# dontLoveBugs/CSPN_monodepth

Hardware: AMD Instinct MI355X
Metric: depth-maps/sec at 304x228 b=24, 24 CSPN iters (higher is better)
Workload: dtype f32

## Files before the change

### cspn_monodepth_amd/_lib.py

```python
import ctypes
import os
import shutil
import subprocess
import threading

_PKG = os.path.dirname(os.path.abspath(__file__))
_ROOT = os.path.dirname(_PKG)
SO_PATH = os.environ.get("CSPN_HIP_LIB") or os.path.join(_PKG, "libcspn_hip.so")
CSRC = os.path.join(_PKG, "csrc")
SOURCES = ("cspn_propagate.hip", "cspn_resident.hip", "cspnk_resident.hip", "cspnk_d2.hip", "cspn_prepare.hip", "cspn_backward.hip", "cspn_metrics.hip", "cspn_metrics_frame.hip", "cspn_debug.hip", "cspn_repair.hip", "pac_conv2d.hip", "pac_conv2d_s2.hip", "cspn_unpool.hip")
HEADERS = (os.path.join(CSRC, "cspn_common.hpp"), os.path.join(CSRC, "cspnk_helpers.hpp"), os.path.join(_ROOT, "include", "cspn_hip.h"))
INCLUDE = os.path.join(_ROOT, "include")

CSPN_F32, CSPN_F16 = 0, 1
ABI_VERSION = 10
BLEND_NONE, BLEND_SPARSE, BLEND_PREMASK = 0, 1, 2

EXPORTS = (
    "cspn_abi_version", "cspn_last_error", "cspn_plan_resolve", "cspn3_prepare", "cspn_pac_prepare",
    "cspn_propagate_workspace_bytes", "cspn_propagate", "cspn_propagate_scored", "cspn_propagate_transposed", "cspn3_propagate_from_guidance",
    "cspn_transpose_weights", "cspn3_resident_plan", "cspn3_resident_workspace_bytes", "cspn3_forward_resident", "cspn3_transposed_resident", "cspn3_transposed_resident_guidance",
    "cspnk_resident_plan", "cspnk_resident_workspace_bytes", "cspnk_forward_resident", "cspnk_forward_resident_history", "cspnk_transposed_resident",
    "cspn_grad_weights", "cspn3_grad_guidance", "cspn_pac_grad_guided", "cspn3_backward_tail",
    "cspn_pac_backward_tail", "cspn_metrics_accumulate", "cspn_metrics_per_frame_workspace_bytes", "cspn_metrics_per_frame", "cspn_meter_update",
    "cspn_pac_out_size", "cspn_pac_force_generic", "cspn_pac_conv2d", "cspn_pac_conv2d_grad_input", "cspn_pac_conv2d_grad_kernel", "cspn_pac_nd2col", "cspn_unpool2d", "cspn_unpool2d_backward", "cspn_debug_set_lds_poison",
)


class cspn_plan(ctypes.Structure):
    _fields_ = [("steps_per_launch", ctypes.c_int), ("tile_w", ctypes.c_int), ("tile_h", ctypes.c_int),
                ("quads_per_thread", ctypes.c_int), ("threads", ctypes.c_int), ("force_scalar", ctypes.c_int)]


class cspn_resident_plan(ctypes.Structure):
    _fields_ = [(n, ctypes.c_int) for n in ("steps_per_phase", "tiles_x", "tiles_y", "tile_w", "tile_h", "quads_per_thread",
                                            "threads", "images_per_launch", "launches", "lds_bytes", "n_cu")] + \
               [("region_over_tile", ctypes.c_float), ("spin_limit", ctypes.c_uint), ("debug_stamps", ctypes.c_void_p),
                ("step_form", ctypes.c_int), ("guard", ctypes.c_int)]


STEP_AUTO, STEP_FMA, STEP_DOT2 = 0, 1, 2


class cspn_conv_geometry(ctypes.Structure):
    _fields_ = [(n, ctypes.c_int) for n in ("kh", "kw", "sh", "sw", "ph", "pw", "dh", "dw", "oph", "opw", "transposed")]


BENCH_UNRELATED = ("pac_conv2d.hip", "pac_conv2d_s2.hip", "cspn_unpool.hip", "cspn_metrics_frame.hip")


def _source_digest(flags, code_only=False):
    import hashlib
    import re
    h = hashlib.sha256(" ".join(flags).encode())
# ... 51 lines not shown
        objs = list(pool.map(compile_one, srcs))
    cmd = [hipcc, "--offload-arch=gfx950", "-shared", "-fPIC", "-o", SO_PATH + ".tmp"] + objs
    if verbose:
        print(" ".join(cmd), flush=True)
    subprocess.check_call(cmd)
    os.replace(SO_PATH + ".tmp", SO_PATH)
    with open(stamp, "w") as fh:
        fh.write(digest + "\n")
    return SO_PATH


_lib = None
_lock = threading.Lock()


def _declare(lib):
    vp, ci, cl, cs = ctypes.c_void_p, ctypes.c_int, ctypes.c_long, ctypes.c_size_t
    lib.cspn_abi_version.restype = ci
    lib.cspn_last_error.restype = ctypes.c_char_p
    lib.cspn_plan_resolve.argtypes = [ci, ci, ci, ci, ci, ci, ctypes.POINTER(cspn_plan), ctypes.POINTER(cspn_plan)]
    lib.cspn3_prepare.argtypes = [vp, ci, cl, cl, ci, ci, ci, ci, vp, ci, vp, vp]
    lib.cspn_pac_prepare.argtypes = [vp, ci, ci, ci, ci, ci, vp, ci, vp]
    lib.cspn_propagate_workspace_bytes.argtypes = [ci, ci, ci, ci, ci, ci]
    lib.cspn_propagate_workspace_bytes.restype = cs
    lib.cspn_propagate.argtypes = [vp, ci, vp, vp, vp, vp, vp, ci, ci, ci, ci, ci, ci, ci, ci,
                                   ctypes.POINTER(cspn_plan), vp]
    lib.cspn_propagate_scored.argtypes = [vp, ci, vp, vp, vp, vp, ci, ci, ci, ci, ci, ci, ci, ci, vp, vp, ci,
                                          ctypes.POINTER(cspn_plan), vp]
    lib.cspn_propagate_transposed.argtypes = [vp, ci, vp, vp, vp, ci, ci, ci, ci, ci, ci, ci, ctypes.POINTER(cspn_plan), vp]
    lib.cspn3_propagate_from_guidance.argtypes = [vp, ci, cl, cl, vp, vp, vp, vp, vp, vp, vp, ci, ci, ci, ci, ci, ci, ci,
                                                  vp, vp, ci,
                                                  ctypes.POINTER(cspn_plan), vp]
    lib.cspn3_resident_plan.argtypes = [ci, ci, ci, ci, ci, ci, ctypes.POINTER(cspn_resident_plan)]
    lib.cspn3_resident_workspace_bytes.argtypes = [ci, ci, ci]
    lib.cspn3_resident_workspace_bytes.restype = cs
    lib.cspn3_forward_resident.argtypes = [vp, cl, cl, vp, vp, vp, vp, vp, vp, vp, ctypes.c_uint, vp, ci, ci, ci, ci, ci, ci, vp, vp, ci,
                                           ctypes.POINTER(cspn_resident_plan), vp]
    lib.cspn3_transposed_resident.argtypes = [vp, vp, vp, vp, vp, ctypes.c_uint, vp, ci, ci, ci, ci, ci, ci,
                                              ctypes.POINTER(cspn_resident_plan), vp]
    lib.cspn3_transposed_resident_guidance.argtypes = [vp, cl, cl, vp, vp, vp, vp, vp, ctypes.c_uint, vp, ci, ci, ci, ci, ci, ci,
                                                       ctypes.POINTER(cspn_resident_plan), vp]
    lib.cspnk_resident_plan.argtypes = [ci, ci, ci, ci, ci, ci, ci, ci, ctypes.POINTER(cspn_resident_plan)]
    lib.cspnk_resident_workspace_bytes.argtypes = [ci, ci, ci, ci]
    lib.cspnk_resident_workspace_bytes.restype = cs
    lib.cspnk_forward_resident.argtypes = [vp, ci, ci, vp, vp, vp, ci, vp, ctypes.c_uint, vp, ci, ci, ci, ci, ci, vp, vp, ci,
                                           ctypes.POINTER(cspn_resident_plan), vp]
    lib.cspnk_forward_resident_history.argtypes = [vp, ci, ci, vp, vp, vp, vp, vp, ctypes.c_uint, vp, ci, ci, ci, ci, ci,
                                                   ctypes.POINTER(cspn_resident_plan), vp]
    lib.cspnk_transposed_resident.argtypes = [vp, ci, ci, vp, vp, ci, vp, vp, vp, ctypes.c_uint, vp, ci, ci, ci, ci, ci,
                                              ctypes.POINTER(cspn_resident_plan), vp]
    lib.cspn_transpose_weights.argtypes = [vp, vp, ci, ci, ci, ci, ci, vp]
    lib.cspn_grad_weights.argtypes = [vp, vp, vp, vp, vp, vp, vp, ci, ci, ci, ci, ci, ci, vp]
    lib.cspn3_grad_guidance.argtypes = [vp, ci, cl, cl, ci, vp, ci, vp, vp, vp, ci, ci, ci, vp]
    lib.cspn_pac_grad_guided.argtypes = [vp, ci, vp, vp, ci, ci, ci, ci, ci, vp]
    lib.cspn3_backward_tail.argtypes = [vp, vp, vp, vp, vp, vp, cl, cl, ci, vp, vp, vp, vp, ci, ci, ci, ci, ci, vp]
    lib.cspn_pac_backward_tail.argtypes = [vp, vp, vp, vp, vp, vp, vp, vp, ci, ci, ci, ci, ci, ci, ci, ci, vp]
    lib.cspn_metrics_accumulate.argtypes = [vp, vp, ci, cs, vp, ci, vp]
    lib.cspn_metrics_per_frame_workspace_bytes.argtypes = [ci, cs]
    lib.cspn_metrics_per_frame_workspace_bytes.restype = cs
    lib.cspn_metrics_per_frame.argtypes = [vp, vp, ci, ci, cs, vp, vp, vp]
    lib.cspn_meter_update.argtypes = [vp, ci, vp, vp]
    geom = ctypes.POINTER(cspn_conv_geometry)
    lib.cspn_pac_out_size.argtypes = [ci, ci, geom, ctypes.POINTER(ci), ctypes.POINTER(ci)]
    lib.cspn_pac_force_generic.argtypes = [ci, ctypes.POINTER(ci)]
    lib.cspn_pac_conv2d.argtypes = [vp, vp, vp, ci, ci, ci, ci, ci, ci, geom, vp]
    lib.cspn_pac_conv2d_grad_input.argtypes = [vp, vp, vp, ci, ci, ci, ci, ci, ci, geom, vp]
# ... 35 lines not shown
```

### cspn_monodepth_amd/csrc/cspn_resident.hip

```cpp
#include "cspn_common.hpp"

#include <atomic>

namespace {

struct ResArgs {
    const float* g;
    long g_bs, g_cs;
    const float* d0;
    const float* sparse;
    float* out;
    float* xbuf;
    unsigned* flags;
    unsigned* status;
    unsigned* host_err;
    int last_chunk;
    unsigned seq;
    float* hist;
    float* w_out;
    float* s_out;
    const float* s_in;
    const float* target;
    double* macc;
    int nslots;
    int B, H, W, Wv, T, S;
    int tw, th, tiles_x, tiles_y;
    int wq, wr, hxw, hyw, dr, ls;
    int b0, nb;
    unsigned spin_limit;
    unsigned long long* dbg;
};

__device__ __forceinline__ void st4_dev(float* base, unsigned elem, float a, float b, float c, float d) {
    const v4f v = {a, b, c, d};
    asm volatile("global_store_dwordx4 %0, %1, %2 sc1" ::"v"(elem * 4u), "v"(v), "s"(base) : "memory");
}
template <typename T>
__device__ __forceinline__ T* uniform_ptr(T* p) {
    const unsigned long long u = reinterpret_cast<unsigned long long>(p);
    const unsigned lo = __builtin_amdgcn_readfirstlane((unsigned)u), hi = __builtin_amdgcn_readfirstlane((unsigned)(u >> 32));
    return reinterpret_cast<T*>(((unsigned long long)hi << 32) | lo);
}
#define GLB __attribute__((address_space(1)))
typedef GLB char* gptr;
__device__ __forceinline__ gptr at32(const float* base, unsigned e) {
    return (gptr) reinterpret_cast<unsigned long long>(base) + (e << 2);
}
__device__ __forceinline__ float4 ld4(gptr p) {
    const v4f v = *reinterpret_cast<const GLB v4f*>(p);
    return make_float4(v.x, v.y, v.z, v.w);
}
__device__ __forceinline__ float ld1(gptr p) { return *reinterpret_cast<const GLB float*>(p); }
__device__ __forceinline__ void st4(gptr p, float4 v) {
    const v4f w = {v.x, v.y, v.z, v.w};
    *reinterpret_cast<GLB v4f*>(p) = w;
}
#ifndef CSPN_RES_HIST_NT
#define CSPN_RES_HIST_NT 1
#endif
#ifndef CSPN_RES_STEP_PIPE
#define CSPN_RES_STEP_PIPE 0
#endif
#ifndef CSPN_RES_PUBLISH_ALL
#define CSPN_RES_PUBLISH_ALL 1
#endif
__device__ __forceinline__ void st4_hist(gptr p, float4 v) {
    const v4f w = {v.x, v.y, v.z, v.w};
    if (CSPN_RES_HIST_NT) __builtin_nontemporal_store(w, reinterpret_cast<GLB v4f*>(p));
    else *reinterpret_cast<GLB v4f*>(p) = w;
}
__device__ __forceinline__ float4 ld4_dev(gptr p) {
    const unsigned long long lo = __hip_atomic_load(reinterpret_cast<const GLB unsigned long long*>(p), __ATOMIC_RELAXED, __HIP_MEMORY_SCOPE_AGENT);
    const unsigned long long hi = __hip_atomic_load(reinterpret_cast<const GLB unsigned long long*>(p) + 1, __ATOMIC_RELAXED, __HIP_MEMORY_SCOPE_AGENT);
    return make_float4(__uint_as_float((unsigned)lo), __uint_as_float((unsigned)(lo >> 32)), __uint_as_float((unsigned)hi),
                       __uint_as_float((unsigned)(hi >> 32)));
}
__device__ __forceinline__ float ld1_dev(gptr p) {
    return __uint_as_float(__hip_atomic_load(reinterpret_cast<const GLB unsigned*>(p), __ATOMIC_RELAXED, __HIP_MEMORY_SCOPE_AGENT));
}

constexpr int RES_THREADS = 512;
constexpr int RES_PP = 16352;

template <int NQ, int NTHREADS, int BLEND, int MODE, int CLEAN, int PAC = 0>
__global__ __launch_bounds__(NTHREADS, NTHREADS / 256) void cspn3_resident(const ResArgs a) {
    static_assert(!PAC || MODE <= 2, "the softmax-weight form has no transposed sweep of its own (the published volume feeds MODE 3)");
    constexpr int R = 1, NT = 8, WIN = 6;
    constexpr bool SCORE = MODE == 1, TRANSG = MODE == 4, TRANS = MODE == 3 || TRANSG, HIST = MODE == 2 || TRANS;
    extern __shared__ __attribute__((aligned(16))) float lds[];
    __shared__ int wg_bad;

    const int tid = threadIdx.x;
    const int tiles_per_img = a.tiles_x * a.tiles_y;
    const int wg_round = a.nb * tiles_per_img;
    const int round = (int)blockIdx.x / wg_round;
    const int tile = xcd_contiguous_id((int)blockIdx.x - round * wg_round, wg_round);
    const int bl = tile / tiles_per_img;
// ... 14 lines not shown
            const unsigned old = __hip_atomic_fetch_add(a.status + 2, 1u, __ATOMIC_RELAXED, __HIP_MEMORY_SCOPE_AGENT);
            if (old + 1u == gridDim.x) {
                __hip_atomic_store(a.status + 2, 0u, __ATOMIC_RELAXED, __HIP_MEMORY_SCOPE_AGENT);
                if (a.host_err && a.last_chunk) __hip_atomic_store(a.host_err + 1, a.seq, __ATOMIC_RELAXED, __HIP_MEMORY_SCOPE_SYSTEM);
            }
        }
    };

    if (b >= a.B) { count_out(); return; }

    const float* __restrict__ din0 = uniform_ptr(a.d0 + (size_t)b * HW);
    const float* __restrict__ spg = BLEND ? uniform_ptr(a.sparse + (size_t)b * HW) : nullptr;

    const int wq = a.wq, wr = a.wr;
    const int sy = tid / wq;
    const int sx = tid - sy * wq;
    const int r0 = sy * NQ;
    const bool exch = a.T > a.S;
    const int rx0 = max(exch ? max(0, x0 - a.tw) : 0, min(x0 - a.hxw, W - 4 * wq));
    const int ry0 = max(exch ? max(0, y0 - a.th) : 0, min(y0 - a.hyw, H - wr));
    const int xq = rx0 + 4 * sx;
    const int yq0 = ry0 + r0;
    const bool x_in = (xq >= 0) && (xq < a.Wv);
    const int nval = a.Wv - xq;
    const int lane = tid & 63;
    const bool fix_left = (sx == 0) || (lane == 0);
    const bool fix_right = (sx == wq - 1) || (lane == 63);

    const int dr = a.dr, ls = a.ls;
    float* const cur = lds;
    float* const nxt = lds + RES_PP;
    const int yd0 = ry0 - R;
    const int xd0 = rx0 - 4;
    float4 st0[NQ + 1];
    unsigned st0_in = 0;
    const int step_r = NTHREADS / wq, step_q = NTHREADS - step_r * wq;
    {
    int row = sy, qx = sx;
#pragma unroll
    for (int u = 0; u <= NQ; ++u) {
        const int y = yd0 + row, x = xd0 + 4 + 4 * qx;
        const bool valid = row < dr;
        const bool in = valid && (y >= 0 && y < H && x >= 0 && x < a.Wv);
        if (in) st0_in |= 1u << u;
        st0[u] = ld4(at32(din0, in ? (unsigned)(y * W + x) : 0u));
        if (TRANS && BLEND) {
            const float4 sp = ld4(at32(spg, in ? (unsigned)(y * W + x) : 0u));
            st0[u].x *= 1.f - sgnf(sp.x); st0[u].y *= 1.f - sgnf(sp.y); st0[u].z *= 1.f - sgnf(sp.z); st0[u].w *= 1.f - sgnf(sp.w);
        }
        row += step_r; qx += step_q;
        if (qx >= wq) { qx -= wq; ++row; }
    }
    }
    float ring0 = 0.f;
    bool ring0_in = false;
    if (tid < dr * 2 * R) {
        const int row = tid / (2 * R), c = tid - row * (2 * R);
        const int lc = (c < R) ? (4 - R + c) : (4 + 4 * wq + (c - R));
        const int y = yd0 + row, x = xd0 + lc;
        ring0_in = (y >= 0 && y < H && x >= 0 && x < a.Wv);
        ring0 = ld1(at32(din0, ring0_in ? (unsigned)(y * W + x) : 0u));
        if (TRANS && BLEND) ring0 *= 1.f - sgnf(ld1(at32(spg, ring0_in ? (unsigned)(y * W + x) : 0u)));
    }

    float wreg[NQ][NT][4];
    unsigned in_img = 0, interior = 0;
// ... 204 lines not shown
    float* hist_step = HIST ? uniform_ptr(a.hist + (size_t)b * HW) : nullptr;
    const int n_phase = (a.T + a.S - 1) / a.S;
    const int tile_global = b * tiles_per_img + trem;
    float own[NQ][4];
    float nbl[NQ], nbr[NQ];

    for (int p = 0; p < n_phase; ++p) {
        const int steps = (a.T - p * a.S) < a.S ? (a.T - p * a.S) : a.S;
        const bool last_phase = (p == n_phase - 1);
        const float* __restrict__ xin = uniform_ptr(a.xbuf + (size_t)((p + 1) & 1) * plane + (size_t)b * HW);
        if (p > 0) {
            int tidp = tid;
            asm volatile("" : "+v"(tidp));
            const int tq_in = min(a.tw, rx0 + 4 * wq - x0) >> 2;
            const int th_in = min(a.th, ry0 + wr - y0);
            const int nl = (x0 - rx0) >> 2;
            const int nside = wq - tq_in;
            const int nrow_t = (y0 - ry0) + R;
            const int n_top = nrow_t * wq;
            const int n_bot = (dr - nrow_t - th_in) * wq;
            const int n_side = th_in * nside;
            const int n_halo = n_top + n_bot + n_side;
            float ring_v = 0.f;
            int ring_at = -1;
            if (tidp < dr * 2 * R) {
                const int row = tidp / (2 * R), c = tidp - row * (2 * R);
                const int lc = (c < R) ? (4 - R + c) : (4 + 4 * wq + (c - R));
                const int y = yd0 + row, x = xd0 + lc;
                const bool in = (y >= 0 && y < H && x >= 0 && x < a.Wv);
                const float v = ld1_dev(at32(xin, in ? (unsigned)(y * W + x) : 0u));
                ring_v = in ? v : 0.f;
                ring_at = row * ls + lc;
            }
            for (int base = 0; base < n_halo; base += 2 * NTHREADS) {
                float4 hv[2];
                int at[2];
#pragma unroll
                for (int u = 0; u < 2; ++u) {
                    const int h = base + u * NTHREADS + tidp;
                    int row, qx;
                    if (h < n_top) { row = h / wq; qx = h - row * wq; }
                    else if (h < n_top + n_bot) { const int h2 = h - n_top; row = h2 / wq; qx = h2 - row * wq; row += nrow_t + th_in; }
                    else {
                        const int h3 = h - n_top - n_bot;
                        const int ns = nside > 0 ? nside : 1;
                        row = h3 / ns;
                        const int c = h3 - row * ns;
                        row += nrow_t;
                        qx = c < nl ? c : c + tq_in;
                    }
                    const int y = yd0 + row, x = xd0 + 4 + 4 * qx;
                    const bool valid = h < n_halo;
                    const bool in = valid && y >= 0 && y < H && x >= 0 && x < a.Wv;
                    const float4 v = ld4_dev(at32(xin, in ? (unsigned)(y * W + x) : 0u));
                    hv[u] = make_float4(in ? v.x : 0.f, in ? v.y : 0.f, in ? v.z : 0.f, in ? v.w : 0.f);
                    at[u] = valid ? row * ls + 4 + 4 * qx : -1;
                }
#pragma unroll
                for (int u = 0; u < 2; ++u)
                    if (at[u] >= 0) *reinterpret_cast<float4*>(&cur[at[u]]) = hv[u];
            }
            if (ring_at >= 0) { cur[ring_at] = ring_v; nxt[ring_at] = 0.f; }
            for (int c = tidp; c < 2 * ls; c += NTHREADS) nxt[(c < ls ? 0 : (dr - 1) * ls - ls) + c] = 0.f;
        }
        __syncthreads();

#pragma unroll
        for (int i = 0; i < NQ; ++i) {
            int drow = r0L + i + R;
            drow = drow < dr ? drow : dr - 1;
            const v4f mid = *(lds_cv4f_ptr)(cur + drow * ls + cb);
            own[i][0] = mid.x; own[i][1] = mid.y; own[i][2] = mid.z; own[i][3] = mid.w;
        }
        if (CSPN_RES_STEP_PIPE) {
#pragma unroll
            for (int i = 0; i < NQ; ++i) { nbl[i] = dpp_from_prev_lane(own[i][3]); nbr[i] = dpp_from_next_lane(own[i][0]); }
        }
        if (BLEND && !TRANS && p == 0) {
#pragma unroll
            for (int i = 0; i < NQ; ++i) {
                if (r0L + i < wr) {
                    float4* slot = reinterpret_cast<float4*>(md_lds + (tid * NQ + i) * 4);
                    const float4 m = *slot;
                    *slot = make_float4(m.x * own[i][0], m.y * own[i][1], m.z * own[i][2], m.w * own[i][3]);
                }
            }
        }
        auto step = [&](auto final_c, auto on_c, auto par_c, int final_par) __attribute__((always_inline)) {
            constexpr bool FINAL = decltype(final_c)::value;
            constexpr int PAR = decltype(par_c)::value;
// ... 147 lines not shown
            if (s < plain_steps) step(std::false_type{}, std::true_type{}, P0{}, 0);
            if (last_phase) step(std::true_type{}, std::true_type{}, P0{}, plain_steps & 1);
        } else {
            for (int s = 0; s < plain_steps; ++s) step(std::false_type{}, std::false_type{}, P0{}, 0);
            if (last_phase) step(std::true_type{}, std::false_type{}, P0{}, 0);
        }
        stamp();
        if (!last_phase) {
            float* __restrict__ xout = uniform_ptr(a.xbuf + (size_t)(p & 1) * plane + (size_t)b * HW);
            if (active) {
                unsigned o0 = (unsigned)(yq0L * W + xqL);
                asm volatile("" : "+v"(o0));
#if !CSPN_RES_PUBLISH_ALL
                auto reg_x0 = [&](int t) { const int xx0 = t * a.tw; return max(max(0, xx0 - a.tw), min(xx0 - a.hxw, W - 4 * wq)); };
                auto reg_y0 = [&](int t) { const int yy0 = t * a.th; return max(max(0, yy0 - a.th), min(yy0 - a.hyw, H - wr)); };
                const int pubL = tx > 0 ? reg_x0(tx - 1) + 4 * wq + 1 : -(1 << 30);
                const int pubR = tx + 1 < a.tiles_x ? reg_x0(tx + 1) - 1 : (1 << 30);
                const int pubT = ty > 0 ? reg_y0(ty - 1) + wr + 1 : -(1 << 30);
                const int pubB = ty + 1 < a.tiles_y ? reg_y0(ty + 1) - 1 : (1 << 30);
                const bool col_read = (xqL < pubL) || (xqL + 3 >= pubR);
#endif
#pragma unroll
                for (int i = 0; i < NQ; ++i) {
#if !CSPN_RES_PUBLISH_ALL
                    const bool read = col_read || (yq0L + i < pubT) || (yq0L + i >= pubB);
#else
                    const bool read = true;
#endif
                    if (((interior >> i) & 1u) && read) st4_dev(xout, o0 + (unsigned)(i * W), own[i][0], own[i][1], own[i][2], own[i][3]);
                }
            }
            asm volatile("s_waitcnt vmcnt(0)" ::: "memory");
            __syncthreads();
            const unsigned want = a.seq + (unsigned)p + 1u;
            if (tid == 0) __hip_atomic_store(a.flags + tile_global, want, __ATOMIC_RELAXED, __HIP_MEMORY_SCOPE_AGENT);
            if (tid < 9 && tid != 4) {
                const int ny = ty + tid / 3 - 1, nx = tx + tid % 3 - 1;
                if (ny >= 0 && ny < a.tiles_y && nx >= 0 && nx < a.tiles_x) {
                    const gptr f = (gptr) reinterpret_cast<unsigned long long>(uniform_ptr(a.flags)) + ((unsigned)(b * tiles_per_img + ny * a.tiles_x + nx) << 2);
                    unsigned spins = 0;
                    while ((int)(__hip_atomic_load(reinterpret_cast<const GLB unsigned*>(f), __ATOMIC_RELAXED, __HIP_MEMORY_SCOPE_AGENT) - want) < 0) {
                        ++spins;
                        if ((spins & 255u) == 0u && __hip_atomic_load(a.status, __ATOMIC_RELAXED, __HIP_MEMORY_SCOPE_AGENT) == a.seq) {
                            wg_bad = 1;
                            break;
                        }
                        if (spins >= a.spin_limit) {
                            __hip_atomic_store(a.status, a.seq, __ATOMIC_RELAXED, __HIP_MEMORY_SCOPE_AGENT);
                            wg_bad = 1;
                            break;
                        }
                        __builtin_amdgcn_s_sleep(2);
                    }
                }
            }
            __syncthreads();
            stamp();
            if (wg_bad) {
                if (tid == 0) {
                    __hip_atomic_store(a.status + 1, 1u, __ATOMIC_RELAXED, __HIP_MEMORY_SCOPE_AGENT);
                    if (a.host_err) __hip_atomic_store(a.host_err, 1u, __ATOMIC_RELAXED, __HIP_MEMORY_SCOPE_SYSTEM);
                    __atomic_thread_fence(__ATOMIC_SEQ_CST);
                }
                {
                    const float qnan = __uint_as_float(CSPN_POISON_F32);
                    float* const pz = HIST ? uniform_ptr(a.hist + (size_t)(a.T - 1) * plane + (size_t)b * HW) : dout;
                    unsigned o0 = (unsigned)(yq0L * W + xqL);
                    asm volatile("" : "+v"(o0));
#pragma unroll
                    for (int i = 0; i < NQ; ++i)
                        if ((interior >> i) & 1u) st4(at32(pz, o0 + (unsigned)(i * W)), make_float4(qnan, qnan, qnan, qnan));
                }
                count_out();
                return;
            }
        }
    }
    if (SCORE) {
        float mf[10];
#pragma unroll
        for (int k = 0; k < 10; ++k) mf[k] = 0.f;
        if (active) {
            float4 scored_t[NQ];
            const float* tgt_b = uniform_ptr(a.target + (size_t)b * HW);
            unsigned o0s = (unsigned)(yq0L * W + xqL);
// ... 30 lines not shown
        }
    }
    count_out();
}

constexpr int RES_MAX_NQ = 5;

constexpr int RES_MAX_ROUNDS = 8;
#ifndef CSPN_RES_ONE_LAUNCH
#define CSPN_RES_ONE_LAUNCH 0
#endif
struct ResGeom {
    int S, tiles_x, tiles_y, tw, th, nq, wq, wr, hxw, hyw, dr, ls;
    int imgs_per_launch, launches;
    size_t lds_bytes;
    double cost;
    int threads = RES_THREADS;
};

int cu_count() {
    static std::atomic<int> cached[64];
    int dev = 0;
    if (hipGetDevice(&dev) != hipSuccess) return 0;
    int n = cached[dev & 63].load(std::memory_order_relaxed);
    if (n > 0) return n;
    hipDeviceProp_t prop;
    if (hipGetDeviceProperties(&prop, dev) != hipSuccess) return 0;
    cached[dev & 63].store(prop.multiProcessorCount, std::memory_order_relaxed);
    return prop.multiProcessorCount;
}

size_t res_lds_bytes(int dr, int ls, int nq, int blend, int threads = RES_THREADS) {
    return ((size_t)RES_PP + (size_t)dr * ls + (size_t)(blend ? 1 : 0) * threads * nq * 4 + 16 * 10) * sizeof(float);
}

#ifndef CSPN_RES_LS_SWIZZLE
#define CSPN_RES_LS_SWIZZLE 1
#endif
int res_row_stride(int wq, int nq, int dr) {
    const int lo = 4 * wq + 8;
    if (!CSPN_RES_LS_SWIZZLE) return lo;
    for (int cand = lo; cand < lo + 64; cand += 4)
        if ((((nq * cand - 4 * wq) % 64) + 64) % 64 == 0 && (size_t)dr * cand <= (size_t)RES_PP) return cand;
    return lo;
}

bool regions_inside_image(const ResGeom& g, int H, int W, int Wv, int T) {
    if (Wv != W) return false;
    const bool exch = T > g.S;
    for (int tx = 0; tx < g.tiles_x; ++tx) {
        const int x0 = tx * g.tw;
        int rx0 = x0 - g.hxw; if (rx0 > W - 4 * g.wq) rx0 = W - 4 * g.wq;
        int lo = exch ? x0 - g.tw : 0; if (lo < 0) lo = 0;
        if (rx0 < lo) rx0 = lo;
        if (rx0 + 4 * g.wq > W) return false;
    }
    for (int ty = 0; ty < g.tiles_y; ++ty) {
        const int y0 = ty * g.th;
        int ry0 = y0 - g.hyw; if (ry0 > H - g.wr) ry0 = H - g.wr;
        int lo = exch ? y0 - g.th : 0; if (lo < 0) lo = 0;
        if (ry0 < lo) ry0 = lo;
        if (ry0 + g.wr > H) return false;
    }
    return true;
}

// ... 79 lines not shown
        if (mode == 2) return launch_resident_inst<NQ, 1, 2, CLEAN>(a, grid, lds, st);
        return mode ? launch_resident_inst<NQ, 1, 1, CLEAN>(a, grid, lds, st) : launch_resident_inst<NQ, 1, 0, CLEAN>(a, grid, lds, st);
    }
    if (mode == 2) return launch_resident_inst<NQ, 0, 2, CLEAN>(a, grid, lds, st);
    return mode ? launch_resident_inst<NQ, 0, 1, CLEAN>(a, grid, lds, st) : launch_resident_inst<NQ, 0, 0, CLEAN>(a, grid, lds, st);
}
template <int NQ>
int launch_resident_nq(const ResArgs& a, int grid, size_t lds, int blend, int mode, bool clean, hipStream_t st) {
    return clean ? launch_resident_c<NQ, 1>(a, grid, lds, blend, mode, st) : launch_resident_c<NQ, 0>(a, grid, lds, blend, mode, st);
}


}

namespace {
int resident_launch(const void* guidance, long bs, long cs, const void* d0, const void* sparse, void* out, void* history,
                    void* w8_out, float* s_out, void* work, unsigned seq, unsigned* host_err, int B, int H, int W, int W_valid,
                    int T, int blend, const void* target, double* acc, int nslots, const cspn_resident_plan* plan,
                    cspn_stream_t stream, bool transposed, bool pac = false, const float* s_in = nullptr);
}

extern "C" {

int cspn3_resident_plan(int B, int H, int W, int T, int blend, int n_cu, cspn_resident_plan* out) {
    if (!out || B < 1 || H < 1 || W < 1 || T < 0) return fail("cspn3_resident_plan: bad arguments");
    if (n_cu <= 0) n_cu = cu_count();
    if (n_cu <= 0) return fail("cspn3_resident_plan: no device (pass n_cu > 0 to plan without one)");
    ResGeom g;
    if (T < 1 || !resident_geometry(B, H, W, T, blend, n_cu, out->steps_per_phase, &g, out->threads))
        return fail("cspn3_resident_plan: no resident tiling for B=%d %dx%d T=%d on %d CUs (W %% 4 == 0 needed)", B, H, W, T, n_cu);
    if (ceil_div(T, g.S) > 255) return fail("cspn3_resident_plan: T=%d in %d-step phases is more than 255 phases", T, g.S);
    out->steps_per_phase = g.S; out->tiles_x = g.tiles_x; out->tiles_y = g.tiles_y; out->tile_w = g.tw; out->tile_h = g.th;
    out->quads_per_thread = g.nq; out->threads = g.threads; out->images_per_launch = g.imgs_per_launch;
    out->launches = g.launches; out->lds_bytes = (int)g.lds_bytes; out->n_cu = n_cu;
    out->region_over_tile = (float)((double)(4 * g.wq) * g.wr / ((double)g.tw * g.th));
    return 1;
}

size_t cspn3_resident_workspace_bytes(int B, int H, int W) {
    const size_t planes = (size_t)2 * B * H * W * sizeof(float);
    const size_t flags = ((size_t)B * (((size_t)H * W) / 16 + 1) + 4) * sizeof(unsigned);
    return ((planes + 15) & ~(size_t)15) + ((flags + 15) & ~(size_t)15);
}

int cspn3_forward_resident(const void* guidance, long bs, long cs, const void* d0, const void* sparse, void* out,
                           void* history, void* w8_out, float* s_out,
                           void* work, unsigned seq, unsigned* host_err, int B, int H, int W, int W_valid, int T, int blend,
                           const void* target, double* acc, int nslots, const cspn_resident_plan* plan,
                           cspn_stream_t stream) {
    return resident_launch(guidance, bs, cs, d0, sparse, out, history, w8_out, s_out, work, seq, host_err, B, H, W, W_valid, T,
                           blend, target, acc, nslots, plan, stream, false);
}

int cspn3_transposed_resident(const void* w8, const float* g_T, const float* sparse_f32, float* history, void* work,
                              unsigned seq, unsigned* host_err, int B, int H, int W, int W_valid, int T, int premask,
                              const cspn_resident_plan* plan, cspn_stream_t stream) {
    if (!w8 || !g_T || !history) return fail("cspn3_transposed_resident: bad arguments");
    if (premask && !sparse_f32) return fail("cspn3_transposed_resident: premask needs sparse");
    return resident_launch(w8, (long)8 * H * W, (long)H * W, g_T, premask ? sparse_f32 : nullptr, nullptr, history, nullptr, nullptr,
                           work, seq, host_err, B, H, W, W_valid, T, premask ? 1 : 0, nullptr, nullptr, 0, plan, stream,
                           true);
}

int cspn3_transposed_resident_guidance(const void* guidance, long bs, long cs, const float* S, const float* g_T,
                                       const float* sparse_f32, float* history, void* work, unsigned seq, unsigned* host_err,
                                       int B, int H, int W, int W_valid, int T, int premask, const cspn_resident_plan* plan,
                                       cspn_stream_t stream) {
    if (!guidance || !S || !g_T || !history) return fail("cspn3_transposed_resident_guidance: bad arguments");
    if (premask && !sparse_f32) return fail("cspn3_transposed_resident_guidance: premask needs sparse");
// ... 52 lines not shown
        g.wq = (g.tw + 2 * g.hxw) / 4; g.wr = g.th + 2 * g.hyw;
        g.dr = g.wr + 2;
        g.threads = rp.threads == 1024 ? 1024 : RES_THREADS;
        g.nq = g.wq > 0 && g.wq <= g.threads ? ceil_div(g.wr, g.threads / g.wq) : RES_MAX_NQ + 1;
        if (g.threads == 1024 && g.nq > 1) g.nq = RES_MAX_NQ + 1;
        g.ls = res_row_stride(g.wq, g.nq, g.dr);
        g.lds_bytes = res_lds_bytes(g.dr, g.ls, g.nq, blend, g.threads);
        g.imgs_per_launch = rp.images_per_launch;
        const int phases = ceil_div(T, Se);
        if ((g.tw & 3) || g.nq > RES_MAX_NQ || g.lds_bytes > 160 * 1024 || (size_t)g.dr * g.ls > (size_t)RES_PP || (phases > 1 && (Se & 1)) || g.tiles_x * g.tw < W || g.tiles_y * g.th < H ||
            (long)g.imgs_per_launch * g.tiles_x * g.tiles_y > ncu ||
            (phases > 1 && ((g.tiles_x > 1 && g.tw < 2 * g.hxw) || (g.tiles_y > 1 && g.th < 2 * g.hyw))))
            return fail("cspn3_forward_resident: the plan does not fit this problem / device (use cspn3_resident_plan)");
    } else if (!resident_geometry(B, H, W, T, blend, ncu, rp.steps_per_phase, &g, rp.threads)) {
        return fail("cspn3_forward_resident: no resident tiling for B=%d %dx%d T=%d", B, H, W, T);
    }
    if (ceil_div(T, g.S) > 255)
        return fail("cspn3_forward_resident: T=%d in %d-step phases is more than 255 phases (use the multi-launch schedule)", T, g.S);
    ResArgs a{};
    a.g = static_cast<const float*>(guidance); a.g_bs = bs; a.g_cs = cs;
    a.d0 = static_cast<const float*>(d0); a.sparse = static_cast<const float*>(sparse); a.out = static_cast<float*>(out);
    const size_t planes = (((size_t)2 * B * H * W * sizeof(float)) + 15) & ~(size_t)15;
    a.xbuf = static_cast<float*>(work);
    a.status = reinterpret_cast<unsigned*>(static_cast<char*>(work) + planes);
    a.flags = a.status + 4;
    if ((size_t)B * g.tiles_x * g.tiles_y > (size_t)B * (((size_t)H * W) / 16 + 1))
        return fail("cspn3_forward_resident: workspace too small for %d tiles", B * g.tiles_x * g.tiles_y);
    a.host_err = host_err;
    a.hist = static_cast<float*>(history); a.w_out = static_cast<float*>(w8_out); a.s_out = s_out;
    if (pac && transposed) return fail("cspn3_forward_resident: the softmax-weight form has no transposed sweep (use cspn3_transposed_resident on the volume)");
    const int mode = transposed ? (s_in ? 7 : 3) : (history ? 2 : (acc ? 1 : 0)) + (pac ? 4 : 0);
    a.s_in = s_in;
    a.seq = seq;
    a.target = static_cast<const float*>(target); a.macc = acc; a.nslots = nslots;
    a.B = B; a.H = H; a.W = W; a.Wv = (W_valid > 0 && W_valid < W) ? W_valid : W; a.T = T; a.S = g.S;
    a.tw = g.tw; a.th = g.th; a.tiles_x = g.tiles_x; a.tiles_y = g.tiles_y;
    a.wq = g.wq; a.wr = g.wr; a.hxw = g.hxw; a.hyw = g.hyw; a.dr = g.dr; a.ls = g.ls;
    a.spin_limit = rp.spin_limit ? rp.spin_limit : (4u << 20);
    a.dbg = rp.debug_stamps;
    const bool clean = regions_inside_image(g, H, W, a.Wv, T);
    if (rp.guard && ((mode != 0 && mode != 1 && mode != 2 && mode != 3 && mode != 7 && mode != 4 && mode != 6) || ((mode == 0 || mode == 1 || mode == 4) && !out) ||
                     !cspn_detail::resident_repair_fits(T)))
        return fail("cspn3_forward_resident: plan->guard serves inference (plain / scored), the training forward and the reverse sweeps, T <= 54 steps");
    const int ipl = g.imgs_per_launch < B ? g.imgs_per_launch : B;
    const int max_rounds = CSPN_RES_ONE_LAUNCH ? RES_MAX_ROUNDS : 1;
    for (int b0 = 0; b0 < B; b0 += ipl * max_rounds) {
        a.b0 = b0;
        a.nb = (B - b0) < ipl ? (B - b0) : ipl;
        const int rounds = ceil_div(B - b0, ipl) < max_rounds ? ceil_div(B - b0, ipl) : max_rounds;
        a.last_chunk = (b0 + ipl * max_rounds >= B) ? 1 : 0;
        const int grid = rounds * a.nb * g.tiles_x * g.tiles_y;
        int ok = 0;
        if (g.threads == 1024) {
            ok = clean ? launch_resident_1024<1>(a, grid, g.lds_bytes, blend, mode, st) : launch_resident_1024<0>(a, grid, g.lds_bytes, blend, mode, st);
            if (!ok) return 0;
            continue;
        }
        switch (g.nq) {
            case 1: ok = launch_resident_nq<1>(a, grid, g.lds_bytes, blend, mode, clean, st); break;
            case 2: ok = launch_resident_nq<2>(a, grid, g.lds_bytes, blend, mode, clean, st); break;
            case 3: ok = launch_resident_nq<3>(a, grid, g.lds_bytes, blend, mode, clean, st); break;
            case 4: ok = launch_resident_nq<4>(a, grid, g.lds_bytes, blend, mode, clean, st); break;
            case 5: ok = launch_resident_nq<5>(a, grid, g.lds_bytes, blend, mode, clean, st); break;
            default: return fail("cspn3_forward_resident: no instance for %d quads per thread", g.nq);
        }
        if (!ok) return 0;
    }
    if (rp.guard)
        return cspn_detail::resident_repair_launch(a.g, bs, cs, a.d0, a.sparse, a.out, a.hist, a.s_out, a.w_out, a.s_in,
                                                   mode == 7 ? 4 : mode == 4 ? 10 : mode == 6 ? 12 : mode, a.status, seq, B, H, W, a.Wv, T, blend ? 1 : 0, ncu, st,
                                                   a.target, a.macc, a.nslots);
    return 1;
}

}
```

### include/cspn_hip.h

```cpp
#ifndef CSPN_HIP_H_
#define CSPN_HIP_H_

#include <stddef.h>

#ifdef __cplusplus
extern "C" {
#endif

#define CSPN_ABI_VERSION 10

#define CSPN_POISON_F32 0x7fc0deadu
#define CSPN_POISON_F16 0x7eadu

typedef void* cspn_stream_t;

enum { CSPN_F32 = 0, CSPN_F16 = 1 };

enum {
    CSPN_BLEND_NONE = 0,
    CSPN_BLEND_SPARSE = 1,
    CSPN_BLEND_PREMASK = 2
};

typedef struct cspn_plan {
// ... 72 lines not shown
int cspn_metrics_per_frame(const void* pred, const void* target, int dtype, int B, size_t pixels_per_frame,
                           void* work, double* sums, cspn_stream_t stream);

int cspn_meter_update(const double* sums, int B, double* meter, cspn_stream_t stream);

typedef struct cspn_conv_geometry {
    int kh, kw;
    int sh, sw;
    int ph, pw;
    int dh, dw;
    int oph, opw;
    int transposed;
} cspn_conv_geometry;

int cspn_pac_out_size(int H, int W, const cspn_conv_geometry* geom, int* Ho, int* Wo);

typedef struct cspn_resident_plan {
    int steps_per_phase;
    int tiles_x, tiles_y;
    int tile_w, tile_h;
    int quads_per_thread, threads;
    int images_per_launch, launches;
    int lds_bytes, n_cu;
    float region_over_tile;
    unsigned spin_limit;
    unsigned long long* debug_stamps;
    int step_form;
    int guard;
} cspn_resident_plan;
#define CSPN_STEP_AUTO 0
#define CSPN_STEP_FMA 1
#define CSPN_STEP_DOT2 2
int cspn3_resident_plan(int B, int H, int W, int T, int blend, int n_cu, cspn_resident_plan* in_out);
size_t cspn3_resident_workspace_bytes(int B, int H, int W);
int cspn3_forward_resident(const void* guidance, long g_batch_stride, long g_chan_stride, const void* d0,
                           const void* sparse_or_null, void* out, void* history_or_null, void* w8_out_or_null,
                           float* s_out_or_null, void* work, unsigned seq, unsigned* host_err_or_null,
                           int B, int H, int W, int W_valid, int T, int blend, const void* target_or_null,
                           double* acc_or_null, int nslots, const cspn_resident_plan* plan_or_null, cspn_stream_t stream);

int cspn3_transposed_resident(const void* w8, const float* g_T, const float* sparse_f32_or_null, float* history, void* work,
                              unsigned seq, unsigned* host_err_or_null, int B, int H, int W, int W_valid, int T, int premask,
                              const cspn_resident_plan* plan_or_null, cspn_stream_t stream);
int cspn3_transposed_resident_guidance(const void* guidance, long g_batch_stride, long g_chan_stride, const float* s,
                                       const float* g_T, const float* sparse_f32_or_null, float* history, void* work,
                                       unsigned seq, unsigned* host_err_or_null, int B, int H, int W, int W_valid, int T,
                                       int premask, const cspn_resident_plan* plan_or_null, cspn_stream_t stream);

int cspnk_resident_plan(int K, int g_dtype, int B, int H, int W, int T, int blend, int n_cu, cspn_resident_plan* in_out);
size_t cspnk_resident_workspace_bytes(int B, int H, int W, int state_dtype);
int cspnk_forward_resident(const void* guided, int g_dtype, int K, const void* x0, const void* sparse_or_null, void* out,
                           int state_dtype, void* work, unsigned seq, unsigned* host_err_or_null, int B, int H, int W,
                           int T, int blend, const void* target_or_null, double* acc_or_null, int nslots,
                           const cspn_resident_plan* plan_or_null, cspn_stream_t stream);
int cspnk_forward_resident_history(const void* guided, int g_dtype, int K, const void* x0, const void* sparse_or_null,
                                   void* history, void* wk_out, void* work, unsigned seq, unsigned* host_err_or_null,
                                   int B, int H, int W, int T, int blend, const cspn_resident_plan* plan_or_null,
                                   cspn_stream_t stream);

int cspnk_transposed_resident(const void* wk, int w_dtype, int K, const void* g_T, const void* sparse_or_null, int in_dtype,
                              float* g_T_f32_out_or_null, float* history, void* work, unsigned seq, unsigned* host_err_or_null,
                              int B, int H, int W, int T, int premask, const cspn_resident_plan* plan_or_null, cspn_stream_t stream);

int cspn_pac_force_generic(int on, int* previous_or_null);

int cspn_pac_conv2d(const void* input, const void* kernel, void* out, int dtype, int B, int C, int kernel_ch,
// ... 20 lines not shown
```

Measured before the change: 527,500.

## Precompute halo exchange index table in LDS and pipeline neighbor flag polling

Builds a per-workgroup LDS table of halo global offsets and LDS destinations once at kernel start, so each phase's halo exchange loads precomputed entries instead of recomputing the divisions and bounds checks. It also replaces the single-load spin wait on neighbor tile flags with several outstanding polls in flight, which is meant to shorten the time spent waiting on inter-workgroup barriers. The table enlarges the LDS allocation and can lower occupancy or fail to fit. It also adds a new exported API for querying the table size.

```diff
diff --git a/cspn_monodepth_amd/_lib.py b/cspn_monodepth_amd/_lib.py
--- a/cspn_monodepth_amd/_lib.py
+++ b/cspn_monodepth_amd/_lib.py
@@ -19,7 +19,7 @@
 EXPORTS = (
     "cspn_abi_version", "cspn_last_error", "cspn_plan_resolve", "cspn3_prepare", "cspn_pac_prepare",
     "cspn_propagate_workspace_bytes", "cspn_propagate", "cspn_propagate_scored", "cspn_propagate_transposed", "cspn3_propagate_from_guidance",
-    "cspn_transpose_weights", "cspn3_resident_plan", "cspn3_resident_workspace_bytes", "cspn3_forward_resident", "cspn3_transposed_resident", "cspn3_transposed_resident_guidance",
+    "cspn_transpose_weights", "cspn3_resident_plan", "cspn3_resident_halo_table_bytes", "cspn3_resident_workspace_bytes", "cspn3_forward_resident", "cspn3_transposed_resident", "cspn3_transposed_resident_guidance",
     "cspnk_resident_plan", "cspnk_resident_workspace_bytes", "cspnk_forward_resident", "cspnk_forward_resident_history", "cspnk_transposed_resident",
     "cspn_grad_weights", "cspn3_grad_guidance", "cspn_pac_grad_guided", "cspn3_backward_tail",
     "cspn_pac_backward_tail", "cspn_metrics_accumulate", "cspn_metrics_per_frame_workspace_bytes", "cspn_metrics_per_frame", "cspn_meter_update",
@@ -137,6 +137,7 @@
                                                   vp, vp, ci,
                                                   ctypes.POINTER(cspn_plan), vp]
     lib.cspn3_resident_plan.argtypes = [ci, ci, ci, ci, ci, ci, ctypes.POINTER(cspn_resident_plan)]
+    lib.cspn3_resident_halo_table_bytes.argtypes = [ci, ci, ci, ci, ci, ci, ctypes.POINTER(cspn_resident_plan)]
     lib.cspn3_resident_workspace_bytes.argtypes = [ci, ci, ci]
     lib.cspn3_resident_workspace_bytes.restype = cs
     lib.cspn3_forward_resident.argtypes = [vp, cl, cl, vp, vp, vp, vp, vp, vp, vp, ctypes.c_uint, vp, ci, ci, ci, ci, ci, ci, vp, vp, ci,
diff --git a/cspn_monodepth_amd/csrc/cspn_resident.hip b/cspn_monodepth_amd/csrc/cspn_resident.hip
--- a/cspn_monodepth_amd/csrc/cspn_resident.hip
+++ b/cspn_monodepth_amd/csrc/cspn_resident.hip
@@ -28,6 +28,7 @@
     int wq, wr, hxw, hyw, dr, ls;
     int b0, nb;
     unsigned spin_limit;
+    int hk;
     unsigned long long* dbg;
 };
 
@@ -63,6 +64,18 @@
 #endif
 #ifndef CSPN_RES_PUBLISH_ALL
 #define CSPN_RES_PUBLISH_ALL 1
+#endif
+#ifndef CSPN_RES_POLL_DEPTH
+#define CSPN_RES_POLL_DEPTH 4
+#endif
+#ifndef CSPN_RES_POLL_GAP
+#define CSPN_RES_POLL_GAP 4
+#endif
+#ifndef CSPN_RES_HALO_TABLE
+#define CSPN_RES_HALO_TABLE 1
+#endif
+#ifndef CSPN_RES_XCHG_STAMPS
+#define CSPN_RES_XCHG_STAMPS 0
 #endif
 __device__ __forceinline__ void st4_hist(gptr p, float4 v) {
     const v4f w = {v.x, v.y, v.z, v.w};
@@ -143,6 +156,34 @@
     float* const nxt = lds + RES_PP;
     const int yd0 = ry0 - R;
     const int xd0 = rx0 - 4;
+    auto halo_table = [&]() { return reinterpret_cast<uint2*>(lds + RES_PP + a.dr * a.ls + (BLEND ? 1 : 0) * NTHREADS * NQ * 4 + 16 * 10); };
+    constexpr bool TBL = CSPN_RES_HALO_TABLE && (NQ < 5 || (!BLEND && MODE <= 1 && !PAC));
+    auto table_in_use = [&]() { return TBL && a.hk > 0; };
+    if (table_in_use()) {
+        uint2* const halo_tbl = halo_table();
+        int wqv = wq, dx0 = x0 - rx0, dy0 = y0 - ry0, twv = a.tw, thv = a.th, wrv = wr, drv = dr;
+        asm volatile("" : "+v"(wqv), "+v"(dx0), "+v"(dy0), "+v"(twv), "+v"(thv), "+v"(wrv), "+v"(drv));
+        const int tq_in = min(twv, 4 * wqv - dx0) >> 2, th_in = min(thv, wrv - dy0);
+        const int nl = dx0 >> 2, nside = wqv - tq_in, nrow_t = dy0 + R;
+        const int n_top = nrow_t * wqv, n_bot = (drv - nrow_t - th_in) * wqv, n_halo = n_top + n_bot + th_in * nside;
+        const int ns = nside > 0 ? nside : 1;
+        const float inv_wq = __builtin_amdgcn_rcpf((float)wqv), inv_ns = __builtin_amdgcn_rcpf((float)ns);
+        for (int k = 0; k < a.hk; ++k) {
+            const int h = k * NTHREADS + tid;
+            const bool side = h >= n_top + n_bot;
+            const int num = side ? h - n_top - n_bot : (h < n_top ? h : h - n_top);
+            const int div = side ? ns : wqv;
+            int q = (int)((float)num * (side ? inv_ns : inv_wq));
+            int rem = num - q * div;
+            if (rem < 0) { --q; rem += div; } else if (rem >= div) { ++q; rem -= div; }
+            const int row = side ? q + nrow_t : (h < n_top ? q : q + nrow_t + th_in);
+            const int qx = side ? (rem < nl ? rem : rem + tq_in) : rem;
+            const int y = yd0 + row, x = xd0 + 4 + 4 * qx;
+            const bool valid = h < n_halo;
+            const bool in = valid && y >= 0 && y < H && x >= 0 && x < a.Wv;
+            halo_tbl[h] = make_uint2(in ? ((unsigned)(y * W + x) | 0x80000000u) : 0u, valid ? (unsigned)(row * ls + 4 + 4 * qx) : 0xffffffffu);
+        }
+    }
     float4 st0[NQ + 1];
     unsigned st0_in = 0;
     const int step_r = NTHREADS / wq, step_q = NTHREADS - step_r * wq;
@@ -413,9 +454,20 @@
                 ring_v = in ? v : 0.f;
                 ring_at = row * ls + lc;
             }
-            for (int base = 0; base < n_halo; base += 2 * NTHREADS) {
+            const bool use_tbl = table_in_use();
+            uint2* const halo_tbl = halo_table();
+            const int n_walk = use_tbl ? a.hk * NTHREADS : n_halo;
+            for (int base = 0; base < n_walk; base += 2 * NTHREADS) {
                 float4 hv[2];
                 int at[2];
+                unsigned oin[2];
+                if (use_tbl) {
+#pragma unroll
+                    for (int u = 0; u < 2; ++u) {
+                        const uint2 e = halo_tbl[base + u * NTHREADS + tidp];
+                        oin[u] = e.x; at[u] = (int)e.y;
+                    }
+                } else {
 #pragma unroll
                 for (int u = 0; u < 2; ++u) {
                     const int h = base + u * NTHREADS + tidp;
@@ -433,10 +485,17 @@
                     const int y = yd0 + row, x = xd0 + 4 + 4 * qx;
                     const bool valid = h < n_halo;
                     const bool in = valid && y >= 0 && y < H && x >= 0 && x < a.Wv;
-                    const float4 v = ld4_dev(at32(xin, in ? (unsigned)(y * W + x) : 0u));
+                    oin[u] = in ? ((unsigned)(y * W + x) | 0x80000000u) : 0u;
+                    at[u] = valid ? row * ls + 4 + 4 * qx : -1;
+                }
+                }
+#pragma unroll
+                for (int u = 0; u < 2; ++u) {
+                    const bool in = (oin[u] >> 31) != 0u;
+                    const float4 v = ld4_dev(at32(xin, oin[u] & 0x7fffffffu));
                     hv[u] = make_float4(in ? v.x : 0.f, in ? v.y : 0.f, in ? v.z : 0.f, in ? v.w : 0.f);
-                    at[u] = valid ? row * ls + 4 + 4 * qx : -1;
-                }
+                }
+                if (CSPN_RES_XCHG_STAMPS && base + 2 * NTHREADS >= n_walk) stamp();
 #pragma unroll
                 for (int u = 0; u < 2; ++u)
                     if (at[u] >= 0) *reinterpret_cast<float4*>(&cur[at[u]]) = hv[u];
@@ -650,25 +709,58 @@
             }
             asm volatile("s_waitcnt vmcnt(0)" ::: "memory");
             __syncthreads();
+            if (CSPN_RES_XCHG_STAMPS) stamp();
             const unsigned want = a.seq + (unsigned)p + 1u;
             if (tid == 0) __hip_atomic_store(a.flags + tile_global, want, __ATOMIC_RELAXED, __HIP_MEMORY_SCOPE_AGENT);
             if (tid < 9 && tid != 4) {
                 const int ny = ty + tid / 3 - 1, nx = tx + tid % 3 - 1;
                 if (ny >= 0 && ny < a.tiles_y && nx >= 0 && nx < a.tiles_x) {
                     const gptr f = (gptr) reinterpret_cast<unsigned long long>(uniform_ptr(a.flags)) + ((unsigned)(b * tiles_per_img + ny * a.tiles_x + nx) << 2);
-                    unsigned spins = 0;
-                    while ((int)(__hip_atomic_load(reinterpret_cast<const GLB unsigned*>(f), __ATOMIC_RELAXED, __HIP_MEMORY_SCOPE_AGENT) - want) < 0) {
-                        ++spins;
-                        if ((spins & 255u) == 0u && __hip_atomic_load(a.status, __ATOMIC_RELAXED, __HIP_MEMORY_SCOPE_AGENT) == a.seq) {
-                            wg_bad = 1;
-                            break;
+                    constexpr int PD = NQ >= 5 ? 1 : CSPN_RES_POLL_DEPTH;
+                    if constexpr (PD == 1) {
+                        unsigned spins = 0;
+                        while ((int)(__hip_atomic_load(reinterpret_cast<const GLB unsigned*>(f), __ATOMIC_RELAXED, __HIP_MEMORY_SCOPE_AGENT) - want) < 0) {
+                            ++spins;
+                            if ((spins & 255u) == 0u && __hip_atomic_load(a.status, __ATOMIC_RELAXED, __HIP_MEMORY_SCOPE_AGENT) == a.seq) {
+                                wg_bad = 1;
+                                break;
+                            }
+                            if (spins >= a.spin_limit) {
+                                __hip_atomic_store(a.status, a.seq, __ATOMIC_RELAXED, __HIP_MEMORY_SCOPE_AGENT);
+                                wg_bad = 1;
+                                break;
+                            }
+                            __builtin_amdgcn_s_sleep(2);
                         }
-                        if (spins >= a.spin_limit) {
-                            __hip_atomic_store(a.status, a.seq, __ATOMIC_RELAXED, __HIP_MEMORY_SCOPE_AGENT);
-                            wg_bad = 1;
-                            break;
+                    } else {
+                        auto poll = [&]() { return __hip_atomic_load(reinterpret_cast<const GLB unsigned*>(f), __ATOMIC_RELAXED, __HIP_MEMORY_SCOPE_AGENT); };
+                        unsigned fv[PD];
+#pragma unroll
+                        for (int k = 0; k < PD; ++k) {
+                            fv[k] = poll();
+                            if (k + 1 < PD) __builtin_amdgcn_s_sleep(CSPN_RES_POLL_GAP);
                         }
-                        __builtin_amdgcn_s_sleep(2);
+                        unsigned spins = 0;
+                        for (bool waiting = true; waiting;) {
+#pragma unroll
+                            for (int k = 0; k < PD; ++k) {
+                                if ((int)(fv[k] - want) >= 0) { waiting = false; break; }
+                                ++spins;
+                                if ((spins & 255u) == 0u && __hip_atomic_load(a.status, __ATOMIC_RELAXED, __HIP_MEMORY_SCOPE_AGENT) == a.seq) {
+                                    wg_bad = 1;
+                                    waiting = false;
+                                    break;
+                                }
+                                if (spins >= a.spin_limit) {
+                                    __hip_atomic_store(a.status, a.seq, __ATOMIC_RELAXED, __HIP_MEMORY_SCOPE_AGENT);
+                                    wg_bad = 1;
+                                    waiting = false;
+                                    break;
+                                }
+                                fv[k] = poll();
+                                __builtin_amdgcn_s_sleep(1);
+                            }
+                        }
                     }
                 }
             }
@@ -765,6 +857,35 @@
 
 size_t res_lds_bytes(int dr, int ls, int nq, int blend, int threads = RES_THREADS) {
     return ((size_t)RES_PP + (size_t)dr * ls + (size_t)(blend ? 1 : 0) * threads * nq * 4 + 16 * 10) * sizeof(float);
+}
+
+int res_halo_entries(int S, int T, int H, int W, int tiles_x, int tiles_y, int tw, int th, int wq, int wr, int hxw, int hyw, int dr, int threads, size_t base_bytes,
+                     int nq, bool plain_inference) {
+    if (!CSPN_RES_HALO_TABLE || T <= S) return 0;
+    if (nq >= 5 && !plain_inference) return 0;
+    int tq_min = 1 << 30, th_min = 1 << 30;
+    for (int tx = 0; tx < tiles_x; ++tx) {
+        const int x0 = tx * tw;
+        int rx0 = x0 - hxw; if (rx0 > W - 4 * wq) rx0 = W - 4 * wq;
+        int lo = x0 - tw; if (lo < 0) lo = 0;
+        if (rx0 < lo) rx0 = lo;
+        int in = rx0 + 4 * wq - x0; if (in > tw) in = tw;
+        in >>= 2;
+        if (in < tq_min) tq_min = in;
+    }
+    for (int ty = 0; ty < tiles_y; ++ty) {
+        const int y0 = ty * th;
+        int ry0 = y0 - hyw; if (ry0 > H - wr) ry0 = H - wr;
+        int lo = y0 - th; if (lo < 0) lo = 0;
+        if (ry0 < lo) ry0 = lo;
+        int in = ry0 + wr - y0; if (in > th) in = th;
+        if (in < th_min) th_min = in;
+    }
+    const long n_halo = (long)dr * wq - (long)tq_min * th_min;
+    if (n_halo <= 0 || n_halo > (long)dr * wq) return 0;
+    int hk = (int)((n_halo + threads - 1) / threads);
+    hk += hk & 1;
+    return base_bytes + (size_t)hk * threads * 8 <= (size_t)160 * 1024 ? hk : 0;
 }
 
 #ifndef CSPN_RES_LS_SWIZZLE
@@ -910,9 +1031,18 @@
     if (ceil_div(T, g.S) > 255) return fail("cspn3_resident_plan: T=%d in %d-step phases is more than 255 phases", T, g.S);
     out->steps_per_phase = g.S; out->tiles_x = g.tiles_x; out->tiles_y = g.tiles_y; out->tile_w = g.tw; out->tile_h = g.th;
     out->quads_per_thread = g.nq; out->threads = g.threads; out->images_per_launch = g.imgs_per_launch;
-    out->launches = g.launches; out->lds_bytes = (int)g.lds_bytes; out->n_cu = n_cu;
+    const int hk = res_halo_entries(g.S, T, H, W, g.tiles_x, g.tiles_y, g.tw, g.th, g.wq, g.wr, g.hxw, g.hyw, g.dr, g.threads, g.lds_bytes, g.nq, !blend);
+    out->launches = g.launches; out->lds_bytes = (int)(g.lds_bytes + (size_t)hk * g.threads * 8); out->n_cu = n_cu;
     out->region_over_tile = (float)((double)(4 * g.wq) * g.wr / ((double)g.tw * g.th));
     return 1;
+}
+
+int cspn3_resident_halo_table_bytes(int B, int H, int W, int T, int blend, int n_cu, const cspn_resident_plan* plan) {
+    if (B < 1 || H < 1 || W < 1 || T < 1) return 0;
+    if (n_cu <= 0) n_cu = cu_count();
+    ResGeom g;
+    if (n_cu <= 0 || !resident_geometry(B, H, W, T, blend, n_cu, plan ? plan->steps_per_phase : 0, &g, plan ? plan->threads : 0)) return 0;
+    return res_halo_entries(g.S, T, H, W, g.tiles_x, g.tiles_y, g.tw, g.th, g.wq, g.wr, g.hxw, g.hyw, g.dr, g.threads, g.lds_bytes, g.nq, !blend) * g.threads * 8;
 }
 
 size_t cspn3_resident_workspace_bytes(int B, int H, int W) {
@@ -1031,11 +1161,13 @@
     const int mode = transposed ? (s_in ? 7 : 3) : (history ? 2 : (acc ? 1 : 0)) + (pac ? 4 : 0);
     a.s_in = s_in;
     a.seq = seq;
+    a.hk = res_halo_entries(g.S, T, H, W, g.tiles_x, g.tiles_y, g.tw, g.th, g.wq, g.wr, g.hxw, g.hyw, g.dr, g.threads, g.lds_bytes, g.nq, !blend && mode <= 1);
     a.target = static_cast<const float*>(target); a.macc = acc; a.nslots = nslots;
     a.B = B; a.H = H; a.W = W; a.Wv = (W_valid > 0 && W_valid < W) ? W_valid : W; a.T = T; a.S = g.S;
     a.tw = g.tw; a.th = g.th; a.tiles_x = g.tiles_x; a.tiles_y = g.tiles_y;
     a.wq = g.wq; a.wr = g.wr; a.hxw = g.hxw; a.hyw = g.hyw; a.dr = g.dr; a.ls = g.ls;
     a.spin_limit = rp.spin_limit ? rp.spin_limit : (4u << 20);
+    const size_t lds_launch = g.lds_bytes + (size_t)a.hk * g.threads * 8;
     a.dbg = rp.debug_stamps;
     const bool clean = regions_inside_image(g, H, W, a.Wv, T);
     if (rp.guard && ((mode != 0 && mode != 1 && mode != 2 && mode != 3 && mode != 7 && mode != 4 && mode != 6) || ((mode == 0 || mode == 1 || mode == 4) && !out) ||
@@ -1051,16 +1183,16 @@
         const int grid = rounds * a.nb * g.tiles_x * g.tiles_y;
         int ok = 0;
         if (g.threads == 1024) {
-            ok = clean ? launch_resident_1024<1>(a, grid, g.lds_bytes, blend, mode, st) : launch_resident_1024<0>(a, grid, g.lds_bytes, blend, mode, st);
+            ok = clean ? launch_resident_1024<1>(a, grid, lds_launch, blend, mode, st) : launch_resident_1024<0>(a, grid, lds_launch, blend, mode, st);
             if (!ok) return 0;
             continue;
         }
         switch (g.nq) {
-            case 1: ok = launch_resident_nq<1>(a, grid, g.lds_bytes, blend, mode, clean, st); break;
-            case 2: ok = launch_resident_nq<2>(a, grid, g.lds_bytes, blend, mode, clean, st); break;
-            case 3: ok = launch_resident_nq<3>(a, grid, g.lds_bytes, blend, mode, clean, st); break;
-            case 4: ok = launch_resident_nq<4>(a, grid, g.lds_bytes, blend, mode, clean, st); break;
-            case 5: ok = launch_resident_nq<5>(a, grid, g.lds_bytes, blend, mode, clean, st); break;
+            case 1: ok = launch_resident_nq<1>(a, grid, lds_launch, blend, mode, clean, st); break;
+            case 2: ok = launch_resident_nq<2>(a, grid, lds_launch, blend, mode, clean, st); break;
+            case 3: ok = launch_resident_nq<3>(a, grid, lds_launch, blend, mode, clean, st); break;
+            case 4: ok = launch_resident_nq<4>(a, grid, lds_launch, blend, mode, clean, st); break;
+            case 5: ok = launch_resident_nq<5>(a, grid, lds_launch, blend, mode, clean, st); break;
             default: return fail("cspn3_forward_resident: no instance for %d quads per thread", g.nq);
         }
         if (!ok) return 0;
diff --git a/include/cspn_hip.h b/include/cspn_hip.h
--- a/include/cspn_hip.h
+++ b/include/cspn_hip.h
@@ -128,6 +128,7 @@
 #define CSPN_STEP_FMA 1
 #define CSPN_STEP_DOT2 2
 int cspn3_resident_plan(int B, int H, int W, int T, int blend, int n_cu, cspn_resident_plan* in_out);
+int cspn3_resident_halo_table_bytes(int B, int H, int W, int T, int blend, int n_cu, const cspn_resident_plan* plan_or_null);
 size_t cspn3_resident_workspace_bytes(int B, int H, int W);
 int cspn3_forward_resident(const void* guidance, long g_batch_stride, long g_chan_stride, const void* d0,
                            const void* sparse_or_null, void* out, void* history_or_null, void* w8_out_or_null,
```

New measurement: 525,700. No clear change (-0.4%).
